# rrwick/Autocycler

Measured on NVIDIA H100. Metric: input-assembly Mbp/sec through compress->unitig GFA, higher is better.
Workload: dtype u64

## Files before the change

autocycler_b200/csrc/backend.h:

```cpp
#pragma once
#include <cstddef>
#include <cstdint>
#include <cstdio>
#include <cstdlib>
#include <cstring>
#include <stdexcept>
#include <string>

extern unsigned long long g_ac_kernel_launches;

#ifdef AC_EMULATE
#define AC_HD inline
#define AC_D inline

template <class T> inline T ac_atomic_cas(T* p, T cmp, T val) { T old = *p; if (old == cmp) *p = val; return old; }
template <class T> inline T ac_atomic_add(T* p, T v) { T old = *p; *p = (T)(old + v); return old; }
template <class T> inline T ac_atomic_or(T* p, T v) { T old = *p; *p = (T)(old | v); return old; }
template <class T> inline T ac_atomic_and(T* p, T v) { T old = *p; *p = (T)(old & v); return old; }
template <class T> inline T ac_atomic_min(T* p, T v) { T old = *p; if (v < old) *p = v; return old; }
template <class T> inline T ac_atomic_max(T* p, T v) { T old = *p; if (v > old) *p = v; return old; }
template <class T> inline T ac_ld_volatile(const T* p) { return *p; }
template <class T> inline T ac_ld_cg(const T* p) { return *p; }
inline void ac_st_stream(uint32_t* p, uint32_t v) { *p = v; }
inline void ac_ld_group(const uint64_t* p, uint64_t out[4]) { out[0] = p[0]; out[1] = p[1]; out[2] = p[2]; out[3] = p[3]; }
inline uint64_t ac_umul64hi(uint64_t a, uint64_t b) { return (uint64_t)(((unsigned __int128)a * b) >> 64); }
inline uint32_t ac_popc(uint32_t v) { return (uint32_t)__builtin_popcount(v); }
inline int ac_ctz(uint32_t v) { return __builtin_ctz(v); }

struct AcStream { int dummy; };

inline void* ac_dev_alloc(size_t bytes) { void* p = malloc(bytes ? bytes : 1); if (!p) throw std::runtime_error("emu alloc failed"); return p; }
inline void ac_dev_free(void* p) { free(p); }
inline void ac_memset(void* p, int v, size_t bytes, AcStream*) { memset(p, v, bytes); }
inline void ac_h2d(void* d, const void* h, size_t bytes, AcStream*) { memcpy(d, h, bytes); }
inline void ac_d2h(void* h, const void* d, size_t bytes, AcStream*) { memcpy(h, d, bytes); }
inline void ac_copy_dd(void* dst, const void* src, size_t bytes, AcStream*) { memcpy(dst, src, bytes); }
inline void ac_sync(AcStream*) {}
inline void* ac_host_alloc(size_t bytes) { return malloc(bytes ? bytes : 1); }
inline void ac_host_free(void* p) { free(p); }
inline int ac_smem_optin() { return 227 * 1024; }
struct AcTimer { explicit AcTimer(AcStream*) {} void stop() {} float ms() const { return 0.f; } };
struct DeviceContext {
    int device; AcStream stream{};
    DeviceContext(int device, void*) : device(device) {}
    void make_current() const {}
};

template <class Body> inline void ac_launch(const char*, AcStream*, const Body& body, uint64_t n);
template <int CTAS, class Body> inline void ac_launch_occ(const char* name, AcStream* st, const Body& body, uint64_t n) { ac_launch(name, st, body, n); }
template <class Body> inline void ac_launch(const char*, AcStream*, const Body& body, uint64_t n) {
    for (uint64_t i = 0; i < n; ++i) body(i);
}
struct AcGridSync { void operator()() const {} };
template <class Body> inline void ac_launch_coop(const char*, AcStream*, const Body& body, uint64_t, uint64_t = 256) { AcGridSync sync; body(0, 1, sync); }

#else
#include <cuda_runtime.h>

#ifdef __CUDACC__
#define AC_HD __host__ __device__ __forceinline__
#define AC_D __device__ __forceinline__
#else
#define AC_HD inline
#define AC_D inline
#endif

#define AC_CUDA_CHECK(expr) do { cudaError_t _e = (expr); if (_e != cudaSuccess) \
    throw std::runtime_error(std::string(#expr) + ": " + cudaGetErrorString(_e)); } while (0)

#ifdef __CUDACC__
AC_D uint64_t ac_atomic_cas(uint64_t* p, uint64_t cmp, uint64_t val) {
    return (uint64_t)atomicCAS((unsigned long long*)p, (unsigned long long)cmp, (unsigned long long)val);
}
AC_D uint32_t ac_atomic_cas(uint32_t* p, uint32_t cmp, uint32_t val) { return atomicCAS(p, cmp, val); }
AC_D uint32_t ac_atomic_add(uint32_t* p, uint32_t v) { return atomicAdd(p, v); }
AC_D uint64_t ac_atomic_add(uint64_t* p, uint64_t v) { return (uint64_t)atomicAdd((unsigned long long*)p, (unsigned long long)v); }
AC_D unsigned long long ac_atomic_add(unsigned long long* p, unsigned long long v) { return atomicAdd(p, v); }
AC_D uint32_t ac_atomic_or(uint32_t* p, uint32_t v) { return atomicOr(p, v); }
AC_D uint32_t ac_atomic_min(uint32_t* p, uint32_t v) { return atomicMin(p, v); }
AC_D uint32_t ac_atomic_max(uint32_t* p, uint32_t v) { return atomicMax(p, v); }
AC_D uint64_t ac_atomic_min(uint64_t* p, uint64_t v) { return (uint64_t)atomicMin((unsigned long long*)p, (unsigned long long)v); }
AC_D uint64_t ac_atomic_max(uint64_t* p, uint64_t v) { return (uint64_t)atomicMax((unsigned long long*)p, (unsigned long long)v); }
template <class T> AC_D T ac_ld_volatile(const T* p) { return *(const volatile T*)p; }
AC_D uint64_t ac_ld_cg(const uint64_t* p) { return (uint64_t)__ldcg(reinterpret_cast<const unsigned long long*>(p)); }
AC_D void ac_ld_group(const uint64_t* p, uint64_t out[4]) {
    asm volatile("ld.global.cg.v2.u64 {%0,%1}, [%2];" : "=l"(out[0]), "=l"(out[1]) : "l"(p) : "memory");
    asm volatile("ld.global.cg.v2.u64 {%0,%1}, [%2];" : "=l"(out[2]), "=l"(out[3]) : "l"(p + 2) : "memory");
// ... 3 lines not shown
AC_D uint32_t ac_popc(uint32_t v) { return (uint32_t)__popc(v); }
AC_D int ac_ctz(uint32_t v) { return __ffs((int)v) - 1; }
AC_D uint64_t ac_atomic_or(uint64_t* p, uint64_t v) { return (uint64_t)atomicOr((unsigned long long*)p, (unsigned long long)v); }
AC_D uint64_t ac_atomic_and(uint64_t* p, uint64_t v) { return (uint64_t)atomicAnd((unsigned long long*)p, (unsigned long long)v); }
#endif

struct AcStream { cudaStream_t s; };

inline void* ac_dev_alloc(size_t bytes) { void* p = nullptr; AC_CUDA_CHECK(cudaMalloc(&p, bytes ? bytes : 1)); return p; }
inline void ac_dev_free(void* p) { if (p) cudaFree(p); }
inline void ac_memset(void* p, int v, size_t bytes, AcStream* st) { AC_CUDA_CHECK(cudaMemsetAsync(p, v, bytes, st->s)); }
inline void ac_h2d(void* d, const void* h, size_t bytes, AcStream* st) { AC_CUDA_CHECK(cudaMemcpyAsync(d, h, bytes, cudaMemcpyHostToDevice, st->s)); }
inline void ac_d2h(void* h, const void* d, size_t bytes, AcStream* st) { AC_CUDA_CHECK(cudaMemcpyAsync(h, d, bytes, cudaMemcpyDeviceToHost, st->s)); }
inline void ac_copy_dd(void* dst, const void* src, size_t bytes, AcStream* st) { AC_CUDA_CHECK(cudaMemcpyAsync(dst, src, bytes, cudaMemcpyDeviceToDevice, st->s)); }
inline void ac_sync(AcStream* st) { AC_CUDA_CHECK(cudaStreamSynchronize(st->s)); }
inline void ac_debug_sync(const char* name, AcStream* st) {
    static const bool on = getenv("AC_SYNC_LAUNCHES") != nullptr;
    if (!on) return;
    const cudaError_t e = cudaStreamSynchronize(st->s);
    if (e != cudaSuccess) throw std::runtime_error(std::string("kernel ") + name + " failed: " + cudaGetErrorString(e));
}
inline void* ac_host_alloc(size_t bytes) { void* p = nullptr; AC_CUDA_CHECK(cudaMallocHost(&p, bytes ? bytes : 1)); return p; }
inline void ac_host_free(void* p) { if (p) cudaFreeHost(p); }
inline uint64_t ac_sm_count() {
    static int sms = 0;
    if (!sms) { int dev = 0; cudaGetDevice(&dev); cudaDeviceGetAttribute(&sms, cudaDevAttrMultiProcessorCount, dev); if (sms <= 0) sms = 132; }
    return (uint64_t)sms;
}
inline int ac_smem_optin() {
    static int optin = -1;
    if (optin < 0) { int dev = 0; AC_CUDA_CHECK(cudaGetDevice(&dev)); AC_CUDA_CHECK(cudaDeviceGetAttribute(&optin, cudaDevAttrMaxSharedMemoryPerBlockOptin, dev)); }
    return optin;
}
class AcTimer {
    cudaEvent_t e0 = nullptr, e1 = nullptr; AcStream* st;
public:
    explicit AcTimer(AcStream* st) : st(st) { AC_CUDA_CHECK(cudaEventCreate(&e0)); AC_CUDA_CHECK(cudaEventCreate(&e1)); AC_CUDA_CHECK(cudaEventRecord(e0, st->s)); }
    AcTimer(const AcTimer&) = delete; AcTimer& operator=(const AcTimer&) = delete;
    ~AcTimer() { cudaEventDestroy(e0); cudaEventDestroy(e1); }
    void stop() { AC_CUDA_CHECK(cudaEventRecord(e1, st->s)); }
    float ms() const { float t = 0.f; AC_CUDA_CHECK(cudaEventElapsedTime(&t, e0, e1)); return t; }
};
struct DeviceContext {
    int device; AcStream stream; bool own_stream = false;
    DeviceContext(int device, void* s) : device(device) {
        int n = 0;
        cudaError_t e = cudaGetDeviceCount(&n);
        if (e != cudaSuccess || n == 0)
            throw std::runtime_error(std::string("autocycler_gpu: no CUDA device available (") + cudaGetErrorString(e) + "); this library has no CPU path");
        AC_CUDA_CHECK(cudaSetDevice(device));
        if (s) stream.s = (cudaStream_t)s;
        else { AC_CUDA_CHECK(cudaStreamCreateWithFlags(&stream.s, cudaStreamNonBlocking)); own_stream = true; }
    }
    DeviceContext(const DeviceContext&) = delete; DeviceContext& operator=(const DeviceContext&) = delete;
    ~DeviceContext() { if (own_stream) { cudaSetDevice(device); cudaStreamDestroy(stream.s); } }
    void make_current() const { AC_CUDA_CHECK(cudaSetDevice(device)); }
};

#ifdef __CUDACC__
#include <cooperative_groups.h>
template <class... P, class... A> inline void ac_launch_kernel(const char* name, AcStream* st, void (*kernel)(P...), dim3 grid, dim3 block, size_t smem, A... args) {
    if (smem > 0) AC_CUDA_CHECK(cudaFuncSetAttribute(kernel, cudaFuncAttributeMaxDynamicSharedMemorySize, (int)smem));
    kernel<<<grid, block, smem, st->s>>>(args...);
    cudaError_t e = cudaGetLastError();
    if (e != cudaSuccess) throw std::runtime_error(std::string("launch ") + name + ": " + cudaGetErrorString(e));
    ++g_ac_kernel_launches;
// ... 134 lines not shown
```

autocycler_b200/csrc/pipeline.cu:

```cuda
#include "pipeline.h"

#include <algorithm>
#include <cmath>
#include <vector>

unsigned long long g_ac_kernel_launches = 0;

#define AC_NONE32 0xFFFFFFFFu
#define AC_CHUNK 32
#define AC_MINCHUNK 128
#define AC_MAX_RANKS 16
#define AC_BOUND_STRIPES 64
#ifndef AC_INSERT_CTAS
#define AC_INSERT_CTAS 2
#endif

struct TableView {
    Slot* slots;
    uint64_t cap;
    const uint64_t* packed;
    const SeqInfo* seqs;
    uint32_t n_seqs;
    uint32_t* count_big;
    uint32_t gb;
// ... 1312 lines not shown
struct GfaView {
    const uint32_t* order; const uint32_t* number_of;
    const UnitigRec* rec; const char* arena; const uint32_t* depth; const uint32_t* next_off; const UStrand* next;
};
struct GfaSizeBody {
    GfaView v; uint32_t n_unitigs; uint32_t* s_size; uint32_t* l_size;
    AC_D void operator()(uint64_t n) const {
        if (n == n_unitigs) { s_size[n] = 0; l_size[n] = 0; return; }
        const uint32_t idx = v.order[n], nl = ac_dec_len((uint32_t)n + 1);
        s_size[n] = 2 + nl + 1 + v.rec[idx].len + 6 + ac_dec_len(v.depth[idx]) + 4;
        uint32_t l = 0;
        for (uint32_t from = idx << 1; from <= (idx << 1 | 1u); ++from)
            for (uint32_t x = v.next_off[from]; x < v.next_off[from + 1]; ++x) l += nl + ac_dec_len(v.number_of[v.next[x] >> 1] + 1) + 11;
        l_size[n] = l;
    }
};
struct GfaSegmentBody {
    GfaView v; const uint32_t* s_off; char* text;
    AC_D void operator()(uint64_t n) const {
        const uint32_t idx = v.order[n];
        char* p = text + s_off[n];
        *p++ = 'S'; *p++ = '\t'; p += ac_put_dec(p, (uint32_t)n + 1); *p++ = '\t';
        p += v.rec[idx].len;
        *p++ = '\t'; *p++ = 'D'; *p++ = 'P'; *p++ = ':'; *p++ = 'f'; *p++ = ':'; p += ac_put_dec(p, v.depth[idx]);
        *p++ = '.'; *p++ = '0'; *p++ = '0'; *p++ = '\n';
    }
};
struct GfaChunkCountBody {
    GfaView v; uint32_t n_unitigs; uint32_t* pieces;
    AC_D void operator()(uint64_t n) const { pieces[n] = n == n_unitigs ? 0u : (v.rec[v.order[n]].len + 63) / 64; }
};
struct GfaSequenceBody {
    GfaView v; uint32_t n_unitigs; const uint32_t* piece_off; const uint32_t* s_off; char* text;
    AC_D void operator()(uint64_t c) const {
        uint32_t lo = 0, hi = n_unitigs;
        while (hi - lo > 1) { const uint32_t mid = (lo + hi) >> 1; if (piece_off[mid] <= c) lo = mid; else hi = mid; }
        const uint32_t idx = v.order[lo], first = ((uint32_t)c - piece_off[lo]) * 64, len = v.rec[idx].len;
        const uint32_t m = len - first < 64 ? len - first : 64;
        const char* src = v.arena + v.rec[idx].seq_off + first;
        char* dst = text + s_off[lo] + 2 + ac_dec_len(lo + 1) + 1 + first;
        for (uint32_t i = 0; i < m; ++i) dst[i] = src[i];
    }
};
struct GfaLinkBody {
    GfaView v; const uint32_t* l_off; char* text;
    AC_D void operator()(uint64_t n) const {
        const uint32_t idx = v.order[n];
        char* p = text + l_off[n];
        for (uint32_t rev = 0; rev < 2; ++rev) {
            const uint32_t from = idx << 1 | rev;
            for (uint32_t x = v.next_off[from]; x < v.next_off[from + 1]; ++x) {
                const UStrand to = v.next[x];
                *p++ = 'L'; *p++ = '\t'; p += ac_put_dec(p, (uint32_t)n + 1); *p++ = '\t'; *p++ = rev ? '-' : '+'; *p++ = '\t';
                p += ac_put_dec(p, v.number_of[to >> 1] + 1); *p++ = '\t'; *p++ = (to & 1u) ? '-' : '+'; *p++ = '\t'; *p++ = '0'; *p++ = 'M'; *p++ = '\n';
            }
        }
    }
};
struct PathLastBody { const uint64_t* path_off; uint8_t* last; AC_D void operator()(uint64_t i) const { if (path_off[i + 1] > path_off[i]) last[path_off[i + 1] - 1] = 1; } };
AC_D uint32_t path_number(const UStrand* path, const uint32_t* number_of, uint64_t x) { return (number_of ? number_of[path[x] >> 1] : path[x] >> 1) + 1; }
struct PathSizeBody {
    const UStrand* path; const uint32_t* number_of; const uint8_t* last; uint64_t steps; uint32_t* p_size;
    AC_D void operator()(uint64_t x) const { p_size[x] = x == steps ? 0u : ac_dec_len(path_number(path, number_of, x)) + 1 + (last[x] ? 0u : 1u); }
};
struct PathTokenBody {
    const UStrand* path; const uint32_t* number_of; uint32_t* dst; uint64_t stride; uint32_t n_ranks; uint64_t first[AC_MAX_RANKS + 1];
    AC_D void operator()(uint64_t x) const {
        uint32_t q = 0; while (q + 1 < n_ranks && first[q + 1] <= x) ++q;
        dst[(uint64_t)q * stride + (x - first[q])] = (number_of[path[x] >> 1] << 1) | (path[x] & 1u);
    }
};
struct PathTextBody {
    const UStrand* path; const uint32_t* number_of; const uint8_t* last; const uint32_t* p_off; char* text;
    AC_D void operator()(uint64_t x) const {
        char* p = text + p_off[x];
        p += ac_put_dec(p, path_number(path, number_of, x)); *p++ = (path[x] & 1u) ? '-' : '+';
        if (!last[x]) *p++ = ',';
    }
};
struct PathLineView { const uint64_t* path_off; uint32_t n_seqs; const uint32_t* p_off; const uint64_t* wrap_off; const uint32_t* pre_len; const uint32_t* suf_len; const char* blob; const uint64_t* blob_off;
                      uint64_t wrap_base; };
struct PathTextFullBody {
    const UStrand* path; const uint32_t* number_of; const uint8_t* last; PathLineView v; char* text;
    AC_D void operator()(uint64_t x) const {
        uint32_t lo = 0, hi = v.n_seqs;
        while (hi - lo > 1) { const uint32_t mid = (lo + hi) >> 1; if (v.path_off[mid] <= x) lo = mid; else hi = mid; }
        char* p = text + (v.wrap_off[lo] - v.wrap_base) + v.pre_len[lo] + v.p_off[x];
        p += ac_put_dec(p, path_number(path, number_of, x)); *p++ = (path[x] & 1u) ? '-' : '+';
        if (!last[x]) *p++ = ',';
    }
};
struct PathWrapBody {
    PathLineView v; char* text;
    AC_D void operator()(uint64_t t) const {
        const uint32_t i = (uint32_t)(t >> 1); const bool suffix = t & 1;
        const char* src = v.blob + v.blob_off[i] + (suffix ? v.pre_len[i] : 0u);
        char* dst = text + (v.wrap_off[i] - v.wrap_base) + (suffix ? v.pre_len[i] + v.p_off[v.path_off[i + 1]] : v.p_off[v.path_off[i]]);
        const uint32_t n = suffix ? v.suf_len[i] : v.pre_len[i];
        for (uint32_t b = 0; b < n; ++b) dst[b] = src[b];
    }
};

struct PathOffBody {
    const SeqInfo* seqs; uint32_t n_seqs; const uint64_t* run_start; uint64_t n_runs; uint64_t* path_off;
    AC_D void operator()(uint64_t i) const {
        if (i == n_seqs) { path_off[i] = n_runs; return; }
        uint64_t lo = 0, hi = n_runs;
        while (lo < hi) { const uint64_t mid = (lo + hi) >> 1; if (run_start[mid] < seqs[i].start) lo = mid + 1; else hi = mid; }
        path_off[i] = lo;
    }
};

struct NeedleSlot { uint64_t w[2]; uint32_t id; uint32_t used; };
template <int WH> struct LiteralScanBody {
    const uint64_t* packed; const SeqInfo* seqs; uint32_t n_seqs; KParams p; uint64_t total;
    const NeedleSlot* table; uint64_t table_mask;
    LiteralHit* hits; uint64_t hit_cap; unsigned long long* n_hits;
    AC_D void operator()(uint64_t i) const {
        uint64_t g = i * 64;
        const uint64_t g1 = (g + 64 < total) ? g + 64 : total;
        uint32_t si = find_seq(seqs, n_seqs, g);
        while (g < g1) {
            const SeqInfo s = seqs[si];
            const uint64_t lo = s.start + s.lead, hi = s.start + s.lead + s.len - p.k;
            if (g > hi || s.len < p.k) { if (si + 1 >= n_seqs) return; ++si; if (seqs[si].start > g) g = seqs[si].start; continue; }
            if (g < lo) g = lo;
            if (g >= g1) return;
            const uint64_t stop = (hi + 1 < g1) ? hi + 1 : g1;
            Key<WH> key = fetch_codes<WH>(packed, g, p);
            for (;;) {
                uint64_t slot = key_hash(key) & table_mask;
                for (;;) {
// ... 107 lines not shown
#endif

enum Mark {
    UPLOAD_BEGIN, UPLOAD_END,
    PACK_BEGIN, PACK_END, SAMPLE_END, INSERT_BEGIN, INSERT_END, TABLE_END,
    RUNS_BEGIN, ADJACENCY_END, BOUNDARIES_END,
    FINISH_BEGIN, UNITIGS_END, SEEDS_END, LINKS_END, SEED_SORT_END, WORK_LIST_END, SIMPLIFY_END, GFA_END,
    ALL_BUT_ARENA, RESULTS_END, N_MARKS
};
enum class Stage { UPLOADED, TABLE, RUNS };

struct DevicePipeline::Impl : DeviceContext {
    uint64_t total = 0; uint32_t n_seqs = 0, k = 0, U = 0, n_chunks = 0; int W = 0;
    DevBuf ascii, seqs, d_wrap_off, d_pre_len, d_suf_len, d_blob, d_blob_off, needles;
    ScratchSet scratch;
    ScratchBuf packed{scratch}, interior8{scratch}, slots{scratch}, pos_slot{scratch}, counters{scratch}, count_big{scratch}, claimed{scratch}, claimed_cnt{scratch}, occ_list{scratch},
        ext_filter{scratch}, hits{scratch};
    ScratchBuf flags8{scratch}, bmask{scratch}, bcount{scratch}, boff{scratch}, run_start{scratch}, run_len{scratch}, run_hs{scratch}, run_ts{scratch};
    ScratchBuf run_uk{scratch}, run_dir{scratch}, is_rep{scratch}, rep_idx{scratch}, run_unitig{scratch}, uid_rep{scratch}, slot_unitig{scratch}, unitigs{scratch}, nchunks{scratch},
        chunk_off{scratch}, partial{scratch}, link_count{scratch}, links{scratch}, sort_a{scratch}, sort_b{scratch}, sort_ra{scratch}, sort_rb{scratch}, rank{scratch}, d_len{scratch},
        d_depth{scratch}, need{scratch}, d_seq_off{scratch}, d_min_fpos{scratch}, d_min_rpos{scratch}, d_arena{scratch}, strand_cnt{scratch}, d_next_off{scratch}, d_next{scratch},
        prev_cnt{scratch}, d_prev_off{scratch}, d_prev{scratch}, d_small{scratch}, d_path{scratch}, d_path_off{scratch}, d_rec{scratch}, num_prefix{scratch}, d_fixed{scratch}, cand_flag{scratch},
        cand_index{scratch}, d_cands{scratch}, d_cand_at{scratch}, d_deps{scratch}, d_spec{scratch};
    ScratchBuf d_pred{scratch}, d_level{scratch}, d_flagmax{scratch}, d_counters64{scratch}, d_dirty{scratch}, d_exhausted{scratch}, d_due{scratch}, d_arena2{scratch}, d_arena3{scratch},
        d_pos{scratch}, sort_c{scratch}, sort_d{scratch};
    ScratchBuf d_pos2{scratch}, gfa_s_size{scratch}, gfa_l_size{scratch}, gfa_p_size{scratch}, gfa_pieces{scratch}, d_last{scratch}, d_totals{scratch}, d_text{scratch}, d_own_off{scratch},
        d_own_last{scratch}, d_own_size{scratch}, d_ptext{scratch};
    ScratchBuf own_entries{scratch}, own_runs{scratch};
    DeviceScan scan;
    PinBuf h_rec, h_depth, h_order, h_order2, h_arena, h_next_off, h_next, h_prev_off, h_prev, h_path, h_path_off, h_run_start, h_run_len;
    PinBuf h_cands, h_deps, h_spec, h_fixed, h_text, h_ptext;
#ifndef AC_EMULATE
    cudaEvent_t ev[N_MARKS];
    Impl(int device, void* stream) : DeviceContext(device, stream) { for (auto& e : ev) AC_CUDA_CHECK(cudaEventCreate(&e)); }
    ~Impl() { cudaSetDevice(device); for (auto& e : ev) cudaEventDestroy(e); }
    void mark(Mark m) { AC_CUDA_CHECK(cudaEventRecord(ev[m], stream.s)); }
    void wait_mark(Mark m) { AC_CUDA_CHECK(cudaEventSynchronize(ev[m])); }
    float between(Mark a, Mark b) { float ms = 0; AC_CUDA_CHECK(cudaEventElapsedTime(&ms, ev[a], ev[b])); return ms; }
#else
    Impl(int device, void* stream) : DeviceContext(device, stream) {}
    void mark(Mark) {}
    void wait_mark(Mark) {}
    float between(Mark, Mark) { return 0.f; }
#endif
    bool arena_pending = false;
    const std::function<void()>* before_results = nullptr;

    std::vector<SeqInfo> host_seqs;
    uint64_t cap = 0, n_windows = 0, n_runs = 0, g_begin = 0, g_end = 0, n_slots_used = 0, n_dotted = 0, n_fwords = 0;
    bool any_dotted = false, is_multi = false, big_counts = false;
    Stage stage = Stage::UPLOADED;
    void require(Stage s, const char* message) const { if (stage < s) throw std::runtime_error(message); }
    TableView table_view() { return TableView{slots.as<Slot>(), cap, packed.as<uint64_t>(), seqs.as<SeqInfo>(), n_seqs, big_counts ? count_big.as<uint32_t>() : nullptr, slot_gpos_bits(total), count_alarm()}; }
    static uint32_t count_alarm() { static const uint32_t a = getenv("AC_COUNT_ALARM") ? (uint32_t)atoi(getenv("AC_COUNT_ALARM")) : AC_SLOT_COUNT_ALARM; return a; }
    template <int W> void local_w(uint32_t seq_lo, uint32_t seq_hi, bool multi);
    template <int W> void insert_w();
    uint64_t safe_cap = 0;
    int table_attempt = 0;
    std::vector<std::pair<const void*, uint64_t>> merged;
    template <int W> void merge_w(const void* dev_ptr, uint64_t n);
    template <int W> void runs_local_w();
    template <int W> void unitigs_w(PipelineResult& out);
    void host_arrays(), paths(), work_list(), simplify(), renumber(), gfa(bool split_paths);
    void results(PipelineResult& out, bool keep_positions, bool fused);
    struct Pending {
        uint64_t n_links = 0, n_cands = 0;
        uint32_t* order_built = nullptr; uint32_t* final_order = nullptr; uint8_t* fix_start = nullptr;
        DevBuf* arena_src = nullptr; uint64_t arena_final = 0;
        bool any_moved = false, gfa_on_device = false, paths_split = false;
        uint64_t bases_removed = 0, gfa_bytes = 0;
    } R;
    void pull_graph(PipelineResult& out, bool keep_positions);
    std::vector<char> path_blob; std::vector<uint32_t> path_pre, path_suf; uint64_t path_wrap_total = 0;
    uint64_t uploaded_bytes = 0;
    uint64_t exp_n = 0, n_own_runs = 0; uint32_t own_seq_lo = 0, own_seq_hi = 0; bool exp_valid = false;
    template <int W> uint64_t list_claimed(bool with_filter);
    template <int W> uint64_t count_entries_w();
#ifdef AC_EMULATE
    static void fill(DevBuf* b) { static const bool on = getenv("AC_EMU_POISON") != nullptr; if (on && b->p) memset(b->p, 0xA5, b->cap); }
    void poison() { for (DevBuf* b : scratch.bufs) fill(b); for (DevBuf& b : scan.serial.level) fill(&b); }
    void poison_table() { for (DevBuf* b : {&slots, &pos_slot, &claimed, &claimed_cnt, &occ_list, &count_big, &counters}) fill(b); }
#else
    void poison() {}
    void poison_table() {}
#endif
};

DevicePipeline::DevicePipeline(int device, void* stream) : impl(new Impl(device, stream)) { impl->before_results = &before_results; }
DevicePipeline::~DevicePipeline() { delete impl; }

unsigned long long DevicePipeline::kernel_launches() const { return g_ac_kernel_launches; }
DeviceContext& DevicePipeline::context() { return *impl; }

void DevicePipeline::upload(const uint8_t* ascii, uint64_t total, const SeqInfo* seqs, uint32_t n_seqs, uint32_t k, uint32_t seq_lo, uint32_t seq_hi) {
    Impl& m = *impl; m.make_current();
    if (k < 3 || (k & 1) == 0) throw std::runtime_error("k must be odd and >= 3");
    const int W = (int)((2 * k + 63) / 64);
    if (W > AC_MAX_W) throw std::runtime_error("k-mer sizes above " + std::to_string(AC_MAX_K) + " are not supported by the GPU path (no CPU fallback exists)");
    if (total >= 0xFFFFFFF0ull) throw std::runtime_error("more than 2^32 padded input bytes are not supported");
    if (n_seqs == 0 || total == 0) throw std::runtime_error("no sequences");
    m.total = total; m.n_seqs = n_seqs; m.k = k; m.W = W; m.stage = Stage::UPLOADED;
    m.host_seqs.assign(seqs, seqs + n_seqs);
    m.mark(UPLOAD_BEGIN);
// ... 362 lines not shown
    num_prefix.ensure((size_t)U * 8);
    ac_launch("number_key", &stream, NumberKeyBody{d_rec.as<UnitigRec>(), d_arena.as<char>(), num_prefix.as<uint64_t>()}, U);
    const NumberLess number_less{d_rec.as<UnitigRec>(), d_depth.as<uint32_t>(), d_arena.as<char>(), num_prefix.as<uint64_t>(), nullptr};
    R.order_built = sort_indices(&stream, number_less, U, sort_a.as<uint32_t>(), sort_b.as<uint32_t>(), sort_ra.as<SortRec>(), sort_rb.as<SortRec>());
}

void DevicePipeline::Impl::work_list() {
    d_fixed.ensure((size_t)U * 4); ac_memset(d_fixed.p, 0, (size_t)U * 4, &stream);
    uint8_t* seed_start = d_fixed.as<uint8_t>(); uint8_t* seed_end = seed_start + U; uint8_t* fix_start = R.fix_start = seed_end + U; uint8_t* fix_end = fix_start + U;
    ac_launch("fixed_seed", &stream, FixedSeedBody{d_path_off.as<uint64_t>(), d_path.as<UStrand>(), seed_start, seed_end}, n_seqs);
    ac_copy_dd(fix_start, seed_start, (size_t)U * 2, &stream);
    ac_launch("fixed_spread", &stream, FixedSpreadBody{seed_start, seed_end, d_next_off.as<uint32_t>(), d_next.as<UStrand>(), d_prev_off.as<uint32_t>(), d_prev.as<UStrand>(),
                                                       fix_start, fix_end}, U);
    const CandidateView cview{R.order_built, d_next_off.as<uint32_t>(), d_next.as<UStrand>(), d_prev_off.as<uint32_t>(), d_prev.as<UStrand>(), fix_start, fix_end};
    cand_flag.ensure((2 * (size_t)U + 1) * 4); cand_index.ensure((2 * (size_t)U + 1) * 4);
    ac_launch("candidate_flag", &stream, CandidateFlagBody{cview, U, cand_flag.as<uint32_t>()}, 2ull * U + 1);
    const uint64_t n_cands = R.n_cands = scan(&stream, cand_flag.as<uint32_t>(), cand_index.as<uint32_t>(), 2ull * U + 1);
    d_cands.ensure((n_cands + 1) * sizeof(ExpandCandidate)); d_cand_at.ensure(2 * (size_t)U * 4 + 4); d_deps.ensure((size_t)U * sizeof(ExpandDeps) + 4); d_spec.ensure((n_cands + 1) * 4);
    ac_launch("candidate_fill", &stream, CandidateFillBody{cview, cand_flag.as<uint32_t>(), cand_index.as<uint32_t>(), d_cands.as<ExpandCandidate>(), d_cand_at.as<int32_t>()}, 2ull * U);
    ac_launch("dependents", &stream, DependentsBody{d_next_off.as<uint32_t>(), d_next.as<UStrand>(), d_prev_off.as<uint32_t>(), d_prev.as<UStrand>(), d_cand_at.as<int32_t>(),
                                                    d_deps.as<ExpandDeps>()}, U);
    ac_launch("common_length", &stream, CommonLengthBody{d_cands.as<ExpandCandidate>(), d_rec.as<UnitigRec>(), d_arena.as<char>(), d_spec.as<uint32_t>()}, n_cands);
    mark(WORK_LIST_END);
}

void DevicePipeline::Impl::simplify() {
    const uint64_t n_cands = R.n_cands, arena_bytes = R.arena_final;
    d_pred.ensure(n_cands * 7 * 4); d_level.ensure(n_cands * 4); d_flagmax.ensure(32); d_counters64.ensure((AC_PASS_WORDS + 8) * 8);
    d_dirty.ensure(((n_cands + 63) / 64) * 8 + 8); d_exhausted.ensure(n_cands + 8);
    unsigned long long* c64 = d_counters64.as<unsigned long long>();
    unsigned long long* res = c64 + AC_PASS_WORDS;
    ac_launch("level_pred", &stream, LevelPredBody{d_cands.as<ExpandCandidate>(), d_deps.as<ExpandDeps>(), d_pred.as<int32_t>()}, n_cands);
    ac_memset(d_level.p, 0, n_cands * 4, &stream); ac_memset(d_flagmax.p, 0, 32, &stream);
    ac_launch_coop("levels", &stream, LevelsCoopBody{d_pred.as<int32_t>(), d_level.as<uint32_t>(), d_flagmax.as<uint32_t>(), n_cands}, n_cands, 4096);
    ac_memset(d_counters64.p, 0, (AC_PASS_WORDS + 8) * 8, &stream);
    const RelocBoundBody bound_body{d_cands.as<ExpandCandidate>(), d_rec.as<UnitigRec>(), d_cand_at.as<int32_t>(), c64 + AC_PASS_SET(1) + 1};
    ac_launch("reloc_bound", &stream, bound_body, n_cands);
    uint32_t fm[8]; unsigned long long h64[AC_PASS_WORDS + 8];
    ac_d2h(fm, d_flagmax.p, 32, &stream); ac_d2h(h64, c64, sizeof h64, &stream); ac_sync(&stream);
    if (fm[4]) throw std::runtime_error("candidate levels did not settle");
    unsigned long long bound = 0; for (int x = 0; x < AC_BOUND_STRIPES; ++x) bound += h64[AC_PASS_SET(1) + 1 + x];
    if (arena_bytes + bound >= 0xFFFFFFF0ull) throw std::runtime_error("unitig sequence arena would exceed 4 GB");
    d_arena2.ensure(arena_bytes + 2 * bound + 64);
    ac_copy_dd(d_arena2.p, d_arena.p, arena_bytes, &stream);
    const unsigned long long start = arena_bytes;
    ac_h2d(c64, &start, 8, &stream);
    ac_memset(c64 + AC_PASS_SET(1), 0, AC_PASS_SET_WORDS * 8, &stream);
    ac_memset(d_dirty.p, 0, ((n_cands + 63) / 64) * 8 + 8, &stream); ac_memset(d_exhausted.p, 0, n_cands + 8, &stream);
    static const bool always_grow = getenv("AC_DEVICE_TIGHT_ARENA") != nullptr;
    uint32_t next_set = 0, next_due = 0; uint64_t passes = 0;
    const uint32_t due_stride = fm[3] + 2;
    d_due.ensure((size_t)3 * due_stride * 4); ac_memset(d_due.p, 0, (size_t)3 * due_stride * 4, &stream);
    for (bool first = true;; first = false) {
        const ApplyLevelBody apply{d_cands.as<ExpandCandidate>(), d_deps.as<ExpandDeps>(), d_level.as<uint32_t>(), 0, d_spec.as<uint32_t>(),
                                   d_rec.as<UnitigRec>(), d_arena2.as<char>(), c64, c64, d_dirty.as<uint64_t>(), d_exhausted.as<uint8_t>(), first, c64 + AC_PASS_REMOVED};
        const uint64_t room = always_grow ? 0 : d_arena2.cap;
        ac_launch_coop("simplify", &stream, SimplifyCoopBody{apply, bound_body, n_cands, d_flagmax.as<uint32_t>() + 3, c64, res, room, next_set, first,
                                                             d_due.as<uint32_t>(), due_stride, next_due}, n_cands, 64);
        ac_d2h(h64, c64, sizeof h64, &stream); ac_sync(&stream);
        const unsigned long long* r = h64 + AC_PASS_WORDS;
        R.arena_final = h64[0]; R.bases_removed = h64[AC_PASS_REMOVED]; R.any_moved = r[1] != 0;
        passes += r[2]; next_set = (uint32_t)r[5]; next_due = (uint32_t)r[7];
        if (getenv("AC_HOST_PROFILE")) fprintf(stderr, "[device] expand_repeats launch: %llu passes (%llu so far), %u levels, %llu candidates, %llu left on the work list, last pass moved %llu bases\n",
                                               r[2], (unsigned long long)passes, fm[3], (unsigned long long)n_cands, r[4], r[0]);
        if (r[0] == 0) break;
        if (passes > 1000000) throw std::runtime_error("repeat expansion did not settle");
        bound = r[3];
// ... 14 lines not shown
    R.final_order = sort_indices(&stream, final_less, U, sort_c.as<uint32_t>(), sort_d.as<uint32_t>(), sort_ra.as<SortRec>(), sort_rb.as<SortRec>());
}

void DevicePipeline::Impl::gfa(bool split_paths) {
    d_pos2.ensure((size_t)U * 4);
    ac_launch("inverse_perm", &stream, InversePermBody{R.final_order, d_pos2.as<uint32_t>()}, U);
    const GfaView gv{R.final_order, d_pos2.as<uint32_t>(), d_rec.as<UnitigRec>(), R.arena_src->as<char>(), d_depth.as<uint32_t>(), d_next_off.as<uint32_t>(), d_next.as<UStrand>()};
    gfa_s_size.ensure(((size_t)U + 1) * 4); gfa_l_size.ensure(((size_t)U + 1) * 4); gfa_pieces.ensure(((size_t)U + 1) * 4);
    const uint64_t steps = split_paths ? 0 : n_runs;
    d_last.ensure(steps + 8); gfa_p_size.ensure((steps + 1) * 4);
    ac_launch("gfa_size", &stream, GfaSizeBody{gv, U, gfa_s_size.as<uint32_t>(), gfa_l_size.as<uint32_t>()}, (uint64_t)U + 1);
    ac_launch("gfa_chunk_count", &stream, GfaChunkCountBody{gv, U, gfa_pieces.as<uint32_t>()}, (uint64_t)U + 1);
    d_totals.ensure(64); ac_memset(d_totals.p, 0, 64, &stream);
    if (!split_paths) {
        ac_memset(d_last.p, 0, steps + 8, &stream);
        ac_launch("path_last", &stream, PathLastBody{d_path_off.as<uint64_t>(), d_last.as<uint8_t>()}, n_seqs);
        ac_launch("path_size", &stream, PathSizeBody{d_path.as<UStrand>(), d_pos2.as<uint32_t>(), d_last.as<uint8_t>(), steps, gfa_p_size.as<uint32_t>()}, steps + 1);
        scan.keep_total(&stream, gfa_p_size.as<uint32_t>(), steps + 1, d_totals.as<uint32_t>() + 3);
    }
    scan.keep_total(&stream, gfa_s_size.as<uint32_t>(), (uint64_t)U + 1, d_totals.as<uint32_t>() + 0);
    scan.keep_total(&stream, gfa_l_size.as<uint32_t>(), (uint64_t)U + 1, d_totals.as<uint32_t>() + 1);
    scan.keep_total(&stream, gfa_pieces.as<uint32_t>(), (uint64_t)U + 1, d_totals.as<uint32_t>() + 2);
    uint32_t tot[4];
    ac_d2h(tot, d_totals.p, 16, &stream); ac_sync(&stream);
    const uint64_t s_bytes = tot[0], l_bytes = tot[1], n_pieces = tot[2], p_list_bytes = tot[3];
    char head[64]; const uint64_t head_bytes = (uint64_t)snprintf(head, sizeof head, "H\tVN:Z:1.0\tKM:i:%u\n", k);
    if (path_wrap_total == 0 && n_seqs) throw std::runtime_error("set_path_line_texts() must precede a build that renders the GFA");
    const uint64_t p_bytes = split_paths ? 0 : p_list_bytes + path_wrap_total;
    R.gfa_bytes = head_bytes + s_bytes + l_bytes + p_bytes;
    d_text.ensure(R.gfa_bytes + 64);
    char* text = d_text.as<char>();
    ac_h2d(text, head, head_bytes, &stream);
    ac_launch("gfa_segment", &stream, GfaSegmentBody{gv, gfa_s_size.as<uint32_t>(), text + head_bytes}, U);
    ac_launch("gfa_sequence", &stream, GfaSequenceBody{gv, U, gfa_pieces.as<uint32_t>(), gfa_s_size.as<uint32_t>(), text + head_bytes}, n_pieces);
    ac_launch("gfa_link", &stream, GfaLinkBody{gv, gfa_l_size.as<uint32_t>(), text + head_bytes + s_bytes}, U);
    const PathLineView pv{d_path_off.as<uint64_t>(), n_seqs, gfa_p_size.as<uint32_t>(), d_wrap_off.as<uint64_t>(), d_pre_len.as<uint32_t>(), d_suf_len.as<uint32_t>(),
                          d_blob.as<char>(), d_blob_off.as<uint64_t>(), 0};
    char* p_text = text + head_bytes + s_bytes + l_bytes;
    if (!split_paths) {
        ac_launch("path_text", &stream, PathTextFullBody{d_path.as<UStrand>(), d_pos2.as<uint32_t>(), d_last.as<uint8_t>(), pv, p_text}, steps);
        ac_launch("path_wrap", &stream, PathWrapBody{pv, p_text}, 2ull * n_seqs);
    }
    R.paths_split = split_paths;
    R.gfa_on_device = true;
}

void DevicePipeline::Impl::results(PipelineResult& out, bool keep_positions, bool fused) {
    if (before_results && *before_results) (*before_results)();
    out.fused = fused; out.graph_fetched = false;
    if (fused && !R.gfa_on_device) throw std::runtime_error("fused build: the device GFA writer did not run");
    uint64_t d2h = 0;
    if (R.gfa_on_device) {
        h_text.ensure(R.gfa_bytes + 64);
        ac_d2h(h_text.p, d_text.p, R.gfa_bytes, &stream); d2h += R.gfa_bytes;
    }
    uint32_t small[16];
    ac_d2h(small, d_small.p, 64, &stream); ac_sync(&stream); d2h += 64;
    out.links_single = (R.n_links - small[0]) / 2 + small[0];
    out.length_before = n_slots_used;
    out.length_after = n_slots_used - R.bases_removed;
    out.gfa_text = R.gfa_on_device ? h_text.as<char>() : nullptr; out.gfa_bytes = R.gfa_on_device ? R.gfa_bytes : 0;
    out.n_unitigs = U; out.n_runs = n_runs; out.n_seqs = n_seqs; out.n_links = R.n_links;
    out.h2d_bytes = uploaded_bytes + (uint64_t)n_seqs * sizeof(SeqInfo);
    out.d2h_bytes = d2h;
    if (!fused) pull_graph(out, keep_positions);
    else { mark(ALL_BUT_ARENA); mark(RESULTS_END); arena_pending = true; }
}

void DevicePipeline::Impl::pull_graph(PipelineResult& out, bool keep_positions) {
    const uint64_t n_links = R.n_links, n_cands = R.n_cands; const uint32_t n_strands = 2 * U;
    const uint64_t arena_cap = R.arena_final + R.arena_final / 4 + (1u << 20);
    h_rec.ensure((size_t)U * sizeof(UnitigRec)); h_depth.ensure((size_t)U * 4);
    h_arena.ensure(arena_cap); h_next_off.ensure(((size_t)n_strands + 1) * 4); h_prev_off.ensure(((size_t)n_strands + 1) * 4);
    h_next.ensure(n_links * 4 + 4); h_prev.ensure(n_links * 4 + 4); h_path.ensure(n_runs * 4 + 4); h_path_off.ensure(((size_t)n_seqs + 1) * 8);
    uint64_t d2h = 0;
    auto pull = [&](PinBuf& dst, DevBuf& src, size_t bytes) { if (bytes) ac_d2h(dst.p, src.p, bytes, &stream); d2h += bytes; };
    pull(h_rec, d_rec, (size_t)U * sizeof(UnitigRec)); pull(h_depth, d_depth, (size_t)U * 4);
    const bool plain = !out.fused;
    if (plain) { h_order.ensure((size_t)U * 4 + 4); if (U) { ac_d2h(h_order.p, R.order_built, (size_t)U * 4, &stream); d2h += (size_t)U * 4; } }
    pull(h_next_off, d_next_off, ((size_t)n_strands + 1) * 4); pull(h_prev_off, d_prev_off, ((size_t)n_strands + 1) * 4);
    pull(h_next, d_next, n_links * 4); pull(h_prev, d_prev, n_links * 4); pull(h_path, d_path, n_runs * 4); pull(h_path_off, d_path_off, ((size_t)n_seqs + 1) * 8);
    if (keep_positions) {
        h_run_start.ensure(n_runs * 8 + 8); h_run_len.ensure(n_runs * 4 + 4);
        pull(h_run_start, run_start, n_runs * 8); pull(h_run_len, run_len, n_runs * 4);
    }
    if (plain) {
        h_cands.ensure((n_cands + 1) * sizeof(ExpandCandidate)); h_deps.ensure((size_t)U * sizeof(ExpandDeps) + 4); h_spec.ensure((n_cands + 1) * 4); h_fixed.ensure((size_t)U * 2 + 4);
// ... 34 lines not shown
}

void DevicePipeline::export_path_tokens(void* dst, uint64_t stride, const uint64_t* counts, uint32_t n_ranks) {
    Impl& m = *impl; m.make_current();
    if (m.stage < Stage::RUNS || !m.R.gfa_on_device || !m.R.paths_split) throw std::runtime_error("export_path_tokens follows a finish with split path lines");
    if (n_ranks == 0 || n_ranks > AC_MAX_RANKS) throw std::runtime_error("export_path_tokens: bad rank count");
    PathTokenBody body{m.d_path.as<UStrand>(), m.d_pos2.as<uint32_t>(), (uint32_t*)dst, stride, n_ranks, {0}};
    for (uint32_t q = 0; q < n_ranks; ++q) { if (counts[q] > stride) throw std::runtime_error("export_path_tokens: a rank holds more occurrences than the stride"); body.first[q + 1] = body.first[q] + counts[q]; }
    if (body.first[n_ranks] != m.n_runs) throw std::runtime_error("export_path_tokens: the counts do not add up to the occurrences imported");
    ac_launch("path_tokens", &m.stream, body, m.n_runs);
}
void DevicePipeline::render_path_lines(const void* tokens, uint64_t n_tokens, const char** text, uint64_t* bytes) {
    Impl& m = *impl; m.make_current();
    m.require(Stage::RUNS, "runs_local must precede render_path_lines");
    if (n_tokens != m.n_own_runs) throw std::runtime_error("render_path_lines: one token per occurrence of this rank's sequences is expected");
    if (m.path_pre.size() != m.n_seqs) throw std::runtime_error("set_path_line_texts() must precede render_path_lines");
    const uint32_t lo = m.own_seq_lo, hi = m.own_seq_hi, n_own = hi - lo;
    uint64_t wrap_lo = 0, wrap_hi = 0;
    for (uint32_t i = 0; i < hi; ++i) { const uint64_t b = (uint64_t)m.path_pre[i] + m.path_suf[i]; wrap_hi += b; if (i < lo) wrap_lo += b; }
    uint64_t total_bytes = 0;
    if (n_own) {
        const uint64_t steps = n_tokens;
        m.d_own_off.ensure(((size_t)n_own + 1) * 8); m.d_own_last.ensure(steps + 8); m.d_own_size.ensure((steps + 1) * 4);
        ac_launch("path_off", &m.stream, PathOffBody{m.seqs.as<SeqInfo>() + lo, n_own, m.run_start.as<uint64_t>(), steps, m.d_own_off.as<uint64_t>()}, (uint64_t)n_own + 1);
        ac_memset(m.d_own_last.p, 0, steps + 8, &m.stream);
        ac_launch("path_last", &m.stream, PathLastBody{m.d_own_off.as<uint64_t>(), m.d_own_last.as<uint8_t>()}, n_own);
        ac_launch("path_size", &m.stream, PathSizeBody{(const UStrand*)tokens, nullptr, m.d_own_last.as<uint8_t>(), steps, m.d_own_size.as<uint32_t>()}, steps + 1);
        const uint64_t list_bytes = m.scan(&m.stream, m.d_own_size.as<uint32_t>(), m.d_own_size.as<uint32_t>(), steps + 1);
        total_bytes = list_bytes + (wrap_hi - wrap_lo);
        m.d_ptext.ensure(total_bytes + 64);
        const PathLineView pv{m.d_own_off.as<uint64_t>(), n_own, m.d_own_size.as<uint32_t>(), m.d_wrap_off.as<uint64_t>() + lo, m.d_pre_len.as<uint32_t>() + lo,
                              m.d_suf_len.as<uint32_t>() + lo, m.d_blob.as<char>(), m.d_blob_off.as<uint64_t>() + lo, wrap_lo};
        ac_launch("path_text", &m.stream, PathTextFullBody{(const UStrand*)tokens, nullptr, m.d_own_last.as<uint8_t>(), pv, m.d_ptext.as<char>()}, steps);
        ac_launch("path_wrap", &m.stream, PathWrapBody{pv, m.d_ptext.as<char>()}, 2ull * n_own);
        m.h_ptext.ensure(total_bytes + 64);
        ac_d2h(m.h_ptext.p, m.d_ptext.p, total_bytes, &m.stream);
    }
    ac_sync(&m.stream);
    *text = total_bytes ? m.h_ptext.as<char>() : nullptr; *bytes = total_bytes;
}

void DevicePipeline::build_local(uint32_t seq_lo, uint32_t seq_hi, bool multi) {
    Impl& m = *impl; m.make_current(); const int W = m.W;
    AC_DISPATCH_W(m.local_w, seq_lo, seq_hi, multi)
}
uint64_t DevicePipeline::count_entries() {
    Impl& m = *impl; m.make_current(); const int W = m.W;
    uint64_t count = 0;
    AC_DISPATCH_W(count = m.count_entries_w)
    return count;
}
void DevicePipeline::merge_entries(const void* dev_ptr, uint64_t n) {
    Impl& m = *impl; m.make_current(); const int W = m.W;
    AC_DISPATCH_W(m.merge_w, dev_ptr, n)
}
void DevicePipeline::runs_local() {
    Impl& m = *impl; m.make_current(); const int W = m.W;
    AC_DISPATCH_W(m.runs_local_w)
}
uint64_t DevicePipeline::local_runs() const { return impl->n_runs; }
void DevicePipeline::import_runs_padded(const void* dev_ptr, uint64_t stride, const uint64_t* counts, uint32_t n_ranks) {
    if (n_ranks == 0 || n_ranks > AC_MAX_RANKS) throw std::runtime_error("import_runs_padded: bad rank count");
    const void* ptrs[AC_MAX_RANKS];
    for (uint32_t q = 0; q < n_ranks; ++q) { if (counts[q] > stride) throw std::runtime_error("import_runs_padded: a rank holds more records than the stride"); ptrs[q] = (const char*)dev_ptr + (size_t)q * stride * sizeof(RunRec); }
    import_runs_from(ptrs, counts, n_ranks);
}
const void* DevicePipeline::export_entries_own(uint64_t* n) {
// ... 51 lines not shown
```

Before: 5222.

## Overlap GFA text D2H with rendering and warp-parallelize sequence/wrap copies

Adds a separate non-blocking copy stream and event helpers so segment and link sections of the GFA text are copied to the host while later sections (links, paths) are still being rendered. The sequence and path-wrap copy kernels switch from one thread per piece to one warp per piece, using a ballot-based 32-way search and strided lane copies to coalesce byte traffic. It also lowers the cooperative levels launch block parameter from 4096 to 1024 and adds a profiling script. The extra stream and events add synchronization complexity, and partial copies are ordered only through recorded events.

Measured after the change: 5449 (median of 6 runs). +4.3%, better.

```diff
diff --git a/autocycler_b200/csrc/backend.h b/autocycler_b200/csrc/backend.h
--- a/autocycler_b200/csrc/backend.h
+++ b/autocycler_b200/csrc/backend.h
@@ -53,6 +53,9 @@
 }
 struct AcGridSync { void operator()() const {} };
 template <class Body> inline void ac_launch_coop(const char*, AcStream*, const Body& body, uint64_t, uint64_t = 256) { AcGridSync sync; body(0, 1, sync); }
+struct AcEvent {};
+inline void ac_record(AcEvent*, AcStream*) {}
+inline void ac_wait(AcStream*, AcEvent*) {}
 
 #else
 #include <cuda_runtime.h>
@@ -122,6 +125,14 @@
     if (optin < 0) { int dev = 0; AC_CUDA_CHECK(cudaGetDevice(&dev)); AC_CUDA_CHECK(cudaDeviceGetAttribute(&optin, cudaDevAttrMaxSharedMemoryPerBlockOptin, dev)); }
     return optin;
 }
+struct AcEvent {
+    cudaEvent_t e = nullptr;
+    AcEvent() { AC_CUDA_CHECK(cudaEventCreateWithFlags(&e, cudaEventDisableTiming)); }
+    AcEvent(const AcEvent&) = delete; AcEvent& operator=(const AcEvent&) = delete;
+    ~AcEvent() { cudaEventDestroy(e); }
+};
+inline void ac_record(AcEvent* ev, AcStream* st) { AC_CUDA_CHECK(cudaEventRecord(ev->e, st->s)); }
+inline void ac_wait(AcStream* st, AcEvent* ev) { AC_CUDA_CHECK(cudaStreamWaitEvent(st->s, ev->e, 0)); }
 class AcTimer {
     cudaEvent_t e0 = nullptr, e1 = nullptr; AcStream* st;
 public:
diff --git a/autocycler_b200/csrc/pipeline.cu b/autocycler_b200/csrc/pipeline.cu
--- a/autocycler_b200/csrc/pipeline.cu
+++ b/autocycler_b200/csrc/pipeline.cu
@@ -1368,14 +1368,24 @@
 };
 struct GfaSequenceBody {
     GfaView v; uint32_t n_unitigs; const uint32_t* piece_off; const uint32_t* s_off; char* text;
-    AC_D void operator()(uint64_t c) const {
+    AC_D void operator()(uint64_t t) const {
+        const uint64_t c = t >> 5; const uint32_t lane = (uint32_t)t & 31u;
         uint32_t lo = 0, hi = n_unitigs;
+#ifdef __CUDA_ARCH__
+        while (hi - lo > 1) {
+            const uint32_t step = (hi - lo + 31) / 32, probe = lo + lane * step;
+            const unsigned le = __ballot_sync(0xFFFFFFFFu, probe < hi && piece_off[probe] <= c);
+            lo += (uint32_t)(31 - __clz((int)le)) * step;
+            hi = lo + step < hi ? lo + step : hi;
+        }
+#else
         while (hi - lo > 1) { const uint32_t mid = (lo + hi) >> 1; if (piece_off[mid] <= c) lo = mid; else hi = mid; }
+#endif
         const uint32_t idx = v.order[lo], first = ((uint32_t)c - piece_off[lo]) * 64, len = v.rec[idx].len;
         const uint32_t m = len - first < 64 ? len - first : 64;
         const char* src = v.arena + v.rec[idx].seq_off + first;
         char* dst = text + s_off[lo] + 2 + ac_dec_len(lo + 1) + 1 + first;
-        for (uint32_t i = 0; i < m; ++i) dst[i] = src[i];
+        for (uint32_t i = lane; i < m; i += 32) dst[i] = src[i];
     }
 };
 struct GfaLinkBody {
@@ -1428,12 +1438,13 @@
 };
 struct PathWrapBody {
     PathLineView v; char* text;
-    AC_D void operator()(uint64_t t) const {
+    AC_D void operator()(uint64_t x) const {
+        const uint64_t t = x >> 5; const uint32_t lane = (uint32_t)x & 31u;
         const uint32_t i = (uint32_t)(t >> 1); const bool suffix = t & 1;
         const char* src = v.blob + v.blob_off[i] + (suffix ? v.pre_len[i] : 0u);
         char* dst = text + (v.wrap_off[i] - v.wrap_base) + (suffix ? v.pre_len[i] + v.p_off[v.path_off[i + 1]] : v.p_off[v.path_off[i]]);
         const uint32_t n = suffix ? v.suf_len[i] : v.pre_len[i];
-        for (uint32_t b = 0; b < n; ++b) dst[b] = src[b];
+        for (uint32_t b = lane; b < n; b += 32) dst[b] = src[b];
     }
 };
 
@@ -1607,17 +1618,28 @@
     PinBuf h_cands, h_deps, h_spec, h_fixed, h_text, h_ptext;
 #ifndef AC_EMULATE
     cudaEvent_t ev[N_MARKS];
-    Impl(int device, void* stream) : DeviceContext(device, stream) { for (auto& e : ev) AC_CUDA_CHECK(cudaEventCreate(&e)); }
-    ~Impl() { cudaSetDevice(device); for (auto& e : ev) cudaEventDestroy(e); }
+    AcStream copy_stream;
+    Impl(int device, void* stream) : DeviceContext(device, stream) {
+        for (auto& e : ev) AC_CUDA_CHECK(cudaEventCreate(&e));
+        AC_CUDA_CHECK(cudaStreamCreateWithFlags(&copy_stream.s, cudaStreamNonBlocking));
+    }
+    ~Impl() { cudaSetDevice(device); for (auto& e : ev) cudaEventDestroy(e); cudaStreamDestroy(copy_stream.s); }
     void mark(Mark m) { AC_CUDA_CHECK(cudaEventRecord(ev[m], stream.s)); }
     void wait_mark(Mark m) { AC_CUDA_CHECK(cudaEventSynchronize(ev[m])); }
     float between(Mark a, Mark b) { float ms = 0; AC_CUDA_CHECK(cudaEventElapsedTime(&ms, ev[a], ev[b])); return ms; }
 #else
+    AcStream copy_stream{};
     Impl(int device, void* stream) : DeviceContext(device, stream) {}
     void mark(Mark) {}
     void wait_mark(Mark) {}
     float between(Mark, Mark) { return 0.f; }
 #endif
+    AcEvent text_rendered, text_copied;
+    void copy_text_after_rendering(uint64_t to) {
+        ac_record(&text_rendered, &stream); ac_wait(&copy_stream, &text_rendered);
+        if (to > R.gfa_copied) ac_d2h(h_text.as<char>() + R.gfa_copied, d_text.as<char>() + R.gfa_copied, to - R.gfa_copied, &copy_stream);
+        R.gfa_copied = to;
+    }
     bool arena_pending = false;
     const std::function<void()>* before_results = nullptr;
 
@@ -1643,7 +1665,7 @@
         uint32_t* order_built = nullptr; uint32_t* final_order = nullptr; uint8_t* fix_start = nullptr;
         DevBuf* arena_src = nullptr; uint64_t arena_final = 0;
         bool any_moved = false, gfa_on_device = false, paths_split = false;
-        uint64_t bases_removed = 0, gfa_bytes = 0;
+        uint64_t bases_removed = 0, gfa_bytes = 0, gfa_copied = 0;
     } R;
     void pull_graph(PipelineResult& out, bool keep_positions);
     std::vector<char> path_blob; std::vector<uint32_t> path_pre, path_suf; uint64_t path_wrap_total = 0;
@@ -2072,7 +2094,7 @@
     unsigned long long* res = c64 + AC_PASS_WORDS;
     ac_launch("level_pred", &stream, LevelPredBody{d_cands.as<ExpandCandidate>(), d_deps.as<ExpandDeps>(), d_pred.as<int32_t>()}, n_cands);
     ac_memset(d_level.p, 0, n_cands * 4, &stream); ac_memset(d_flagmax.p, 0, 32, &stream);
-    ac_launch_coop("levels", &stream, LevelsCoopBody{d_pred.as<int32_t>(), d_level.as<uint32_t>(), d_flagmax.as<uint32_t>(), n_cands}, n_cands, 4096);
+    ac_launch_coop("levels", &stream, LevelsCoopBody{d_pred.as<int32_t>(), d_level.as<uint32_t>(), d_flagmax.as<uint32_t>(), n_cands}, n_cands, 1024);
     ac_memset(d_counters64.p, 0, (AC_PASS_WORDS + 8) * 8, &stream);
     const RelocBoundBody bound_body{d_cands.as<ExpandCandidate>(), d_rec.as<UnitigRec>(), d_cand_at.as<int32_t>(), c64 + AC_PASS_SET(1) + 1};
     ac_launch("reloc_bound", &stream, bound_body, n_cands);
@@ -2153,14 +2175,17 @@
     char* text = d_text.as<char>();
     ac_h2d(text, head, head_bytes, &stream);
     ac_launch("gfa_segment", &stream, GfaSegmentBody{gv, gfa_s_size.as<uint32_t>(), text + head_bytes}, U);
-    ac_launch("gfa_sequence", &stream, GfaSequenceBody{gv, U, gfa_pieces.as<uint32_t>(), gfa_s_size.as<uint32_t>(), text + head_bytes}, n_pieces);
+    ac_launch("gfa_sequence", &stream, GfaSequenceBody{gv, U, gfa_pieces.as<uint32_t>(), gfa_s_size.as<uint32_t>(), text + head_bytes}, 32 * n_pieces);
+    h_text.ensure(R.gfa_bytes + 64);
+    copy_text_after_rendering(head_bytes + s_bytes);
     ac_launch("gfa_link", &stream, GfaLinkBody{gv, gfa_l_size.as<uint32_t>(), text + head_bytes + s_bytes}, U);
+    copy_text_after_rendering(head_bytes + s_bytes + l_bytes);
     const PathLineView pv{d_path_off.as<uint64_t>(), n_seqs, gfa_p_size.as<uint32_t>(), d_wrap_off.as<uint64_t>(), d_pre_len.as<uint32_t>(), d_suf_len.as<uint32_t>(),
                           d_blob.as<char>(), d_blob_off.as<uint64_t>(), 0};
     char* p_text = text + head_bytes + s_bytes + l_bytes;
     if (!split_paths) {
         ac_launch("path_text", &stream, PathTextFullBody{d_path.as<UStrand>(), d_pos2.as<uint32_t>(), d_last.as<uint8_t>(), pv, p_text}, steps);
-        ac_launch("path_wrap", &stream, PathWrapBody{pv, p_text}, 2ull * n_seqs);
+        ac_launch("path_wrap", &stream, PathWrapBody{pv, p_text}, 64ull * n_seqs);
     }
     R.paths_split = split_paths;
     R.gfa_on_device = true;
@@ -2172,8 +2197,9 @@
     if (fused && !R.gfa_on_device) throw std::runtime_error("fused build: the device GFA writer did not run");
     uint64_t d2h = 0;
     if (R.gfa_on_device) {
-        h_text.ensure(R.gfa_bytes + 64);
-        ac_d2h(h_text.p, d_text.p, R.gfa_bytes, &stream); d2h += R.gfa_bytes;
+        copy_text_after_rendering(R.gfa_bytes);
+        ac_record(&text_copied, &copy_stream); ac_wait(&stream, &text_copied);
+        d2h += R.gfa_bytes;
     }
     uint32_t small[16];
     ac_d2h(small, d_small.p, 64, &stream); ac_sync(&stream); d2h += 64;
@@ -2274,7 +2300,7 @@
         const PathLineView pv{m.d_own_off.as<uint64_t>(), n_own, m.d_own_size.as<uint32_t>(), m.d_wrap_off.as<uint64_t>() + lo, m.d_pre_len.as<uint32_t>() + lo,
                               m.d_suf_len.as<uint32_t>() + lo, m.d_blob.as<char>(), m.d_blob_off.as<uint64_t>() + lo, wrap_lo};
         ac_launch("path_text", &m.stream, PathTextFullBody{(const UStrand*)tokens, nullptr, m.d_own_last.as<uint8_t>(), pv, m.d_ptext.as<char>()}, steps);
-        ac_launch("path_wrap", &m.stream, PathWrapBody{pv, m.d_ptext.as<char>()}, 2ull * n_own);
+        ac_launch("path_wrap", &m.stream, PathWrapBody{pv, m.d_ptext.as<char>()}, 64ull * n_own);
         m.h_ptext.ensure(total_bytes + 64);
         ac_d2h(m.h_ptext.p, m.d_ptext.p, total_bytes, &m.stream);
     }
diff --git a/profiles/tail_profile.py b/profiles/tail_profile.py
--- /dev/null
+++ b/profiles/tail_profile.py
@@ -0,0 +1,90 @@
+import argparse
+import json
+import os
+import statistics
+import sys
+
+ROOT = os.path.dirname(os.path.dirname(os.path.abspath(__file__)))
+sys.path.insert(0, ROOT)
+
+
+def short_name(name):
+    if "<" in name:
+        inner = name[name.index("<") + 1:]
+        depth, out = 1, []
+        for ch in inner:
+            depth += ch == "<"
+            depth -= ch == ">"
+            if depth == 0 or (depth == 1 and ch == ","):
+                break
+            out.append(ch)
+        return "".join(out).strip()
+    return name.split("(")[0]
+
+
+def main():
+    ap = argparse.ArgumentParser()
+    ap.add_argument("--workload", default="cfg2")
+    ap.add_argument("--k", type=int, default=51)
+    ap.add_argument("--steps", type=int, default=5)
+    ap.add_argument("--warmup", type=int, default=3)
+    ap.add_argument("--out", required=True)
+    args = ap.parse_args()
+    import torch
+    from torch.profiler import ProfilerActivity, profile
+    import bench
+    from autocycler_b200 import api, synth
+    if not torch.cuda.is_available():
+        raise SystemExit("tail_profile.py: no CUDA device")
+    gpu = bench.gpu_identity(0)
+    assemblies = synth.make_assemblies(args.workload)
+    stream = torch.cuda.Stream(device=0)
+    torch.cuda.set_stream(stream)
+    _, seqs, count = bench.prepare_sequences(assemblies, args.k)
+    kg = api.KmerGraph(args.k, device=0, stream=stream.cuda_stream)
+    kg.add_sequences(seqs, count, upload=False)
+    kg.upload()
+    for _ in range(args.warmup):
+        api.UnitigGraph.compress(kg)
+    torch.cuda.synchronize()
+    with profile(activities=[ProfilerActivity.CUDA]) as prof:
+        for _ in range(args.steps):
+            api.UnitigGraph.compress(kg)
+            torch.cuda.synchronize()
+    events = []
+    for e in prof.events():
+        if e.device_type != torch.autograd.DeviceType.CUDA:
+            continue
+        start = e.time_range.start
+        events.append((start, e.time_range.end, short_name(e.name)))
+    events.sort()
+    starts = [i for i, ev in enumerate(events) if ev[2] == "RunKeyBody"]
+    steps = []
+    for si, i0 in enumerate(starts):
+        i1 = starts[si + 1] if si + 1 < len(starts) else len(events)
+        seg = events[i0:i1]
+        last = max(j for j, ev in enumerate(seg) if ev[2].startswith(("Gfa", "Path")))
+        while last + 1 < len(seg) and seg[last + 1][2].startswith("Memcpy"):
+            last += 1
+        seg = seg[:last + 1]
+        rows, prev_end = [], seg[0][0]
+        for s, t, nm in seg:
+            rows.append({"name": nm, "us": round(t - s, 2), "gap_us": round(s - prev_end, 2), "start_us": round(s - seg[0][0], 2)})
+            prev_end = max(prev_end, t)
+        steps.append({"rows": rows, "span_us": round(prev_end - seg[0][0], 2)})
+    os.makedirs(args.out, exist_ok=True)
+    path = os.path.join(args.out, f"tail_{args.workload}.json")
+    json.dump({"gpu": gpu, "workload": args.workload, "k": args.k, "steps": steps}, open(path, "w"), indent=1)
+    same = [st for st in steps if [r["name"] for r in st["rows"]] == [r["name"] for r in steps[0]["rows"]]]
+    print(f"# {args.workload}, k={args.k}: {gpu['name']} at {gpu['power_limit_w']} W; {len(same)} of {len(steps)} steps alike; "
+          f"tail span median {statistics.median(st['span_us'] for st in steps):.1f} us")
+    print("| # | kernel / copy | us | gap before (us) | start (us) |")
+    print("|---|---|---|---|---|")
+    for j, r in enumerate(same[0]["rows"] if same else []):
+        med = lambda key: statistics.median(st["rows"][j][key] for st in same)
+        print(f"| {j} | {r['name']} | {med('us'):.1f} | {med('gap_us'):.1f} | {med('start_us'):.1f} |")
+    print(f"wrote {path}")
+
+
+if __name__ == "__main__":
+    main()
```
